# peterWon/LVI-ExC

Hardware: AMD Instinct MI355X
Metric: M residual+Jacobian evals/s per GN iter (higher is better)
Workload: dtype f64; 1 GPU; config4-full-LVI: 1000000 surfel + 200000 IMU samples (gyro+accel blocks) + 49992 ORB reprojection blocks, 25023 knots @ dt=0.02; step = residuals + analytic Jacobians + Huber + J^T J/J^T r assembly (no linear solve); n_tangent=155259, bandwidth=179, n_border=52, tracks=orb, parallelism=sequence-per-gpu x1, allreduce_transport=none (one sequence)

## Files before the change

### lvi-exc_amd/csrc/lvx_eval.hip

```cpp
#include <algorithm>
#include <cmath>
#include <cstring>
#include <functional>
#include <numeric>
#include <cstdlib>

#include <thread>
#include "lvx_ctx.h"
#include "lvx_fold.h"

namespace lvx {

#define LVX_PW 4
struct Keys { int k0, k1, lm; };
LVX_HD bool same(const Keys& a, const Keys& b) { return a.k0 == b.k0 && a.k1 == b.k1 && a.lm == b.lm; }

struct Cal { ImuCal imu; SensorCal lidar, cam; const double* rho; };
__device__ __forceinline__ Cal load_cal(const DevCommon& cm) {
  const double* s = cm.state + 7 * (size_t)cm.N;
  Cal c;
  c.imu.tau = s[7]; c.imu.roll = s[8]; c.imu.pitch = s[9]; c.imu.ba = load_v3(s + 10); c.imu.bg = load_v3(s + 13);
  c.lidar.q = load_q(s + 16); c.lidar.p = load_v3(s + 20); c.lidar.tau = s[23];
  c.cam.q = load_q(s + 24); c.cam.p = load_v3(s + 28); c.cam.tau = s[31];
  c.rho = s + 32;
// ... 277 lines not shown
      for (int a = 0; a < NR; ++a) {
        int32_t* jc = cm.jcols + (orow + a) * LVX_JAC_WIDTH;
        double* jv = cm.jvals + (orow + a) * LVX_JAC_WIDTH;
#pragma unroll
        for (int c = 0; c < NC; ++c) {
          const int g = fam.col(c, key, cm.N);
          const bool dead = tangent_locked(g, cm.N, cm.L, cm.locks);
          jc[c] = dead ? -1 : g;
          jv[c] = dead ? 0.0 : J[a][c];
        }
        for (int c = NC; c < LVX_JAC_WIDTH; ++c) { jc[c] = -1; jv[c] = 0.0; }
      }
    }
    if (scale != 1.0) {
#pragma unroll
      for (int a = 0; a < NR; ++a) {
        r[a] *= scale;
#pragma unroll
        for (int c = 0; c < NC; ++c) J[a][c] *= scale;
      }
    }
  }
  mycost = wave_sum(mycost);
  if (lane == 0) atomicAdd(&cm.cost[rep], mycost);
  if (cm.what & LVX_EVAL_NORMAL_EQ) {
#pragma unroll
    for (int a = 0; a < NR; ++a) {
      rs[lane * NR + a] = valid ? r[a] : 0.0;
#pragma unroll
      for (int c = 0; c < NC; ++c) Jt[c * TS + lane * NR + a] = valid ? J[a][c] : 0.0;
    }
    Keys pk;
    pk.k0 = __shfl_up(key.k0, 1); pk.k1 = __shfl_up(key.k1, 1); pk.lm = __shfl_up(key.lm, 1);
    const bool head = (lane == 0) || !same(pk, key);
    const unsigned long long heads = __ballot(head);
    const int myseg = __popcll(heads & ((2ull << lane) - 1ull)) - 1;
    if (head) { seg_l0[myseg] = lane; seg_ok[myseg] = valid ? 1 : 0; seg_keys[myseg] = key; }
    if (lane == 0) nseg_s = __popcll(heads);
  }
  }
  if (!(cm.what & LVX_EVAL_NORMAL_EQ)) return;
  __syncthreads();
  const int nseg = nseg_s;
  const int tid = threadIdx.x;
  constexpr int NT = 64 * PW;
  for (int e = tid; e < nseg * NC; e += NT) { const int sg = e / NC, c = e % NC; cpos[e] = seg_ok[sg] ? cm.ord[fam.col(c, seg_keys[sg], cm.N)] : LVX_DEAD; }
  constexpr int ITER = (NP + NC + NT - 1) / NT;
  unsigned code[ITER];
#pragma unroll
  for (int i = 0; i < ITER; ++i) { const int p = tid + NT * i; code[i] = p < NP ? pairs[p] : 0u; }
  __syncthreads();
  for (int sg = 0; sg < nseg; ++sg) {
    if (!seg_ok[sg]) continue;
    const int l0 = seg_l0[sg];
    const int l1 = sg + 1 < nseg ? seg_l0[sg + 1] : 64;
    const int rb = l0 * NR, re = l1 * NR;
    const int* cp = &cpos[sg * NC];
#pragma unroll
    for (int i = 0; i < ITER; ++i) {
      const int p = tid + NT * i;
      if (p < NP) {
        const int a = code[i] & 0xff, b = code[i] >> 8;
        const int pa = cp[a], pb = cp[b];
        if (pa == LVX_DEAD || pb == LVX_DEAD) continue;
        const double* ja = &Jt[a * TS];
        const double* jb = &Jt[b * TS];
        double acc = 0.0;
        for (int row = rb; row < re; ++row) acc += ja[row] * jb[row];
        if (a != b && pa == pb) acc *= 2.0;
        add_H(cm, pa, pb, acc, rep);
      } else if (p < NP + NC) {
        const int c = p - NP;
        const int pc = cp[c];
        if (pc == LVX_DEAD) continue;
        const double* jc = &Jt[c * TS];
        double acc = 0.0;
        for (int row = rb; row < re; ++row) acc += jc[row] * rs[row];
        add_g(cm, pc, acc, rep);
      }
    }
  }
}

__device__ void hub_eval_thread(const DevCommon& cm, double t_map, int want_surf, int want_cs, HubShared* hubs, int s) {
  if (s > 1) return;
  if ((s == 0 && !want_surf) || (s == 1 && !want_cs)) { hubs[s].ok = 0; return; }
#ifdef LVX_KTIME_FOLD
  long long kt_[5] = {0, 0, 0, 0, 0}; long long kt0_ = __builtin_amdgcn_s_memtime(); const long long kts_ = kt0_;
#define HKT(i) { const long long n_ = __builtin_amdgcn_s_memtime(); kt_[i] += n_ - kt0_; kt0_ = n_; }
#else
#define HKT(i)
#endif
  const SplineRef sp{cm.t0, cm.dt, cm.N, cm.state, cm.state + 3 * (size_t)cm.N};
  const Cal cal = load_cal(cm);
  const bool tl = s == 0 ? (cm.locks & LVX_LOCK_LIDAR_TAU) != 0 : (cm.locks & LVX_LOCK_CAM_TAU) != 0;
  const double tau = s == 0 ? cal.lidar.tau : cal.cam.tau;
  double s1[1][2]; hub_spans(t_map, tl, cm.sensor_mto, s1);
  HKT(0)
  Segs sg; KnotRef kh; hubs[s].ok = 0;
  if (!build_segments(sp, s1, 1, &sg)) return;
  if (!seg_lookup(sp, sg, t_map + tau, &kh)) return;
  HKT(1)
  if (!(tl ? pose_eval<true>(sp, kh, &hubs[s].A) : pose_eval<true, true>(sp, kh, &hubs[s].A))) { hubs[s].ok = -RES_NONUNIT; return; }
  HKT(2)
  hub_matrix(hubs[s].A, hubs[s].M);
  hubs[s].ok = 1;
  HKT(3)
#ifdef LVX_KTIME_FOLD
  printf("HKT hub set %d: cal+spans %lld segments+lookup %lld pose_eval %lld hub_matrix+stores %lld | total %lld, ends at %lld (ticks of s_memtime)\n", s, kt_[0], kt_[1], kt_[2], kt_[3],
         (long long)__builtin_amdgcn_s_memtime() - kts_, (long long)__builtin_amdgcn_s_memtime());
#endif
}
__device__ __forceinline__ void state_prepass_block(const DevCommon& cm, So3Pre* tab, int nblk_tab, double t_map, int want_surf, int want_cs, HubShared* hubs, int blk) {
  if (blk >= nblk_tab) { hub_eval_thread(cm, t_map, want_surf, want_cs, hubs, threadIdx.x); return; }
  const int k = blk * blockDim.x + threadIdx.x;
  if (k >= cm.N) return;
  const double* so3 = cm.state + 3 * (size_t)cm.N;
  So3Pre e;
  if (k + 1 < cm.N) so3_pre(load_q(so3 + 4 * (size_t)k), load_q(so3 + 4 * (size_t)(k + 1)), &e);
  else { e.Om = mk(0, 0, 0); e.on = 0.0; e.Jri = m3_identity(); e.c3 = 1.0 / 12.0; e.ok = 1; }
  tab[k] = e;
}

struct Aux { int wid, xk, lm; const PreWin* pw; };
struct GyroAcc {
  enum { PMAJ = 1 };
  enum { NK = 12, NG = 3, NR = 3, HUB = -1, KPK = 3, LVO = 3, WS = 1, GL = 32, SKIP_GG = 0, SECONDARY = 0, LB = 64, NCP = 15, USE_PRE = 1, OCC = 1, FAM = LVX_FAM_GYRO };
  __device__ static constexpr int jm(int c) { return c; }
  int n; const double* t; const double* m3; const int* perm; double weight, huber;
  __device__ int eval(const DevCommon& cm, const SplineRef& sp, const Cal& cal, const HubShared*, int si, double r[NR], double (*J)[NCP], int& key, Aux& aux) const {
    return gyro_residual<true, true>(sp, cal.imu, t[si], load_v3(m3 + 3 * (size_t)si), weight, &key, r, J, aux.pw);
  }
  __device__ static int klv(int c) { return 6 * (c / 3) + 3 + c % 3; }
  __device__ static int gcol(int g, int N, int nt) { return 6 * N + 5 + g; }
  __device__ void put(const DevCommon& cm, const HubShared*, int si, bool valid, int key, const double (*J)[NCP]) const {
    if (!valid) { put_skipped(cm, FAM, perm[si]); return; }
    put_record<NR, GYRO_NC>(cm, FAM, perm[si], key, -1, -1, [&](int a, int c) { return J[a][c]; });
  }
};
#ifndef LVX_SURF_WS
#define LVX_SURF_WS 3
#endif
template <bool TAU> struct SurfAccT {
  enum { DEPG = LVX_SURF_WS >= 3 ? 3 : 0 };
  enum { NK = 24, NG = 12 + (TAU ? 1 : 0), NR = 1, HUB = 0, KPK = 6, LVO = 0, WS = LVX_SURF_WS, GL = 16, SKIP_GG = 0, SECONDARY = 0, LB = 64, NCP = 36 + (TAU ? 1 : 0), USE_PRE = 1, OCC = 2, FAM = LVX_FAM_SURFEL };
  __device__ static constexpr int jm(int c) { return c; }
  int n; const double* t; const double* pt; const double* rowpl; const int* perm; double t_map, weight, huber;
  struct Row { double t; v3 p, Pi; };
  enum { PREFETCH = 1 };
  __device__ Row load(int si) const { return Row{t[si], load_v3(pt + 3 * (size_t)si), load_v3(rowpl + 3 * (size_t)si)}; }
  __device__ int eval_row(const DevCommon& cm, const SplineRef& sp, const Cal& cal, const HubShared* hub, const Row& row, double r[NR], double (*J)[NCP], int& key, Aux& aux) const {
    const bool tl = (cm.locks & LVX_LOCK_LIDAR_TAU) != 0;
    const double tk = row.t;
    Segs segs;
    if (tl) {
      KnotRef kr;
      const int st = two_point_lookup(sp, t_map, tk, tk + cal.lidar.tau, &kr);
      if (st >= 0) {
        if (st == 1) return RES_RANGE;
        if (hub->ok != 1) return hub->ok < 0 ? RES_NONUNIT : RES_RANGE;
        if (st == 2) return RES_RANGE;
        LVX_KT(aux.pw, 8)
        return surfel_residual_pseudo<true, TAU>(sp, hub->A, segs, cal.lidar, tk, row.p, row.Pi, weight, &key, r, J, aux.pw, &kr);
      }
    }
    const double pad = tl ? 0.0 : cm.sensor_mto;
    const double spans[2][2] = {{t_map - pad, t_map + pad}, {tk - pad, tk + pad}};
    if (!build_segments(sp, spans, 2, &segs)) return RES_RANGE;
    KnotRef kh;
    if (!seg_lookup(sp, segs, t_map + cal.lidar.tau, &kh)) return RES_RANGE;
    if (hub->ok != 1) return hub->ok < 0 ? RES_NONUNIT : RES_RANGE;
    if (kh.i0 != hub->A.k.i0 || kh.u != hub->A.k.u) return LVX_ERR_FALLBACK;
    LVX_KT(aux.pw, 8)
    return surfel_residual_pseudo<true, TAU>(sp, hub->A, segs, cal.lidar, tk, row.p, row.Pi, weight, &key, r, J, aux.pw);
  }
  __device__ static int klv(int c) { return c; }
  __device__ static int gcol(int g, int N, int nt) { return g < 6 ? nt + g : 6 * N + 8 + (g - 6); }
  __device__ void put(const DevCommon& cm, const HubShared* hub, int si, bool valid, int key, const double (*J)[NCP]) const {
    if (!valid) { put_skipped(cm, FAM, perm[si]); return; }
    put_record<NR, SURF_NC + (TAU ? 1 : 0)>(cm, FAM, perm[si], hub->A.k.i0, key, -1, [&](int a, int c) { return c < 24 ? hub_col(*hub, &J[a][24], c) : (c < 48 ? J[a][c - 24] : J[a][c - 18]); });
  }
};
using SurfAcc = SurfAccT<false>;
template <bool TAU> struct CamSurfAccT {
  enum { NK = 24, NG = 18 + (TAU ? 1 : 0), NR = 1, HUB = 1, KPK = 6, LVO = 0, WS = 1, GL = 16, SKIP_GG = 0, SECONDARY = 0, LB = 64, NCP = 42 + (TAU ? 1 : 0), USE_PRE = 1, OCC = 2, FAM = LVX_FAM_CAMSURF };
  __device__ static constexpr int jm(int c) { return c; }
  int n; const int* lm; const int* plane; const int* perm; const double* planes; const double* lm_uv; const double* lm_t0; double t_map, weight, huber;
  __device__ int eval(const DevCommon& cm, const SplineRef& sp, const Cal& cal, const HubShared* hub, int si, double r[NR], double (*J)[NCP], int& key, Aux& aux) const {
    const bool tl = (cm.locks & LVX_LOCK_CAM_TAU) != 0;
    const int l = lm[si];
    const double tk = lm_t0[l];
    Segs segs;
    if (tl) {
      KnotRef kr;
      const int st = two_point_lookup(sp, t_map, tk, tk + cal.cam.tau, &kr);
      if (st >= 0) {
        if (st == 1) return RES_RANGE;
// ... 140 lines not shown
#pragma unroll
        for (int c = 0; c < 12; ++c) v[c] = src[(size_t)c * n];
      }
      const int k0 = in ? k0r : -1, k1 = in ? k1r : -1;
      const bool live = in && k1 >= 0;
      const int o0 = k0 - 4 * w0, o1 = k1 - 4 * w1;
      const bool stray = live && (o0 < 0 || o0 > 3 || o1 < 0 || o1 > 3);
      const bool valid = live && !stray;
#pragma unroll
      for (int c = 0; c < 12; ++c) v[c] = live ? v[c] : 0.0;
      for (int e = lane; e < 2 * BR * LDP; e += 64) Pr[e] = 0.0;
      __builtin_amdgcn_fence(__ATOMIC_RELEASE, "wavefront");
      __builtin_amdgcn_wave_barrier();
      {
        double* dst = (side ? Po : Pr) + (2 * b + a) * LDP + 6 * (side ? o1 : o0) + 12 * h;
        if (valid) {
#pragma unroll
          for (int c = 0; c < 12; ++c) dst[c] = v[c];
        }
      }
      __builtin_amdgcn_fence(__ATOMIC_RELEASE, "wavefront");
      __builtin_amdgcn_wave_barrier();
      __builtin_amdgcn_fence(__ATOMIC_ACQUIRE, "wavefront");
      const int nks = (2 * min(8, m1 - base) + 3) >> 2;
      for (int ks = 0; ks < nks; ++ks) {
        double fr[3], fo[3];
#pragma unroll
        for (int c = 0; c < 3; ++c) { fr[c] = Pr[ks * 4 * LDP + frag_off + c * 16]; fo[c] = Po[ks * 4 * LDP + frag_off + c * 16]; }
#pragma unroll
        for (int ci = 0; ci < 3; ++ci)
#pragma unroll
          for (int cj = 0; cj < 3; ++cj) D[ci * 3 + cj] = __builtin_amdgcn_mfma_f64_16x16x4f64(fr[ci], fo[cj], D[ci * 3 + cj], 0, 0, 0);
      }
      {
        unsigned long long sm = __ballot(stray && part == 0);
        while (sm) {
          const int sl = __ffsll((long long)sm) - 1; sm &= sm - 1;
          const int sb = sl >> 3;
          const int sk0 = __shfl(k0, sl), sk1 = __shfl(k1, sl);
          __builtin_amdgcn_wave_barrier();
          if (b == sb) {
#pragma unroll
            for (int c = 0; c < 12; ++c) sbuf[wv][a][24 * side + 12 * h + c] = v[c];
          }
          __builtin_amdgcn_fence(__ATOMIC_RELEASE, "wavefront");
          __builtin_amdgcn_wave_barrier();
          __builtin_amdgcn_fence(__ATOMIC_ACQUIRE, "wavefront");
          for (int e2 = lane; e2 < 576; e2 += 64) {
            const int x = e2 / 24, y = e2 % 24;
            const double val = sbuf[wv][0][x] * sbuf[wv][0][24 + y] + sbuf[wv][1][x] * sbuf[wv][1][24 + y];
            if (val == 0.0) continue;
            const int pa = cm.ord[6 * (sk0 + x / 6) + x % 6], pb = cm.ord[6 * (sk1 + y / 6) + y % 6];
            if (pa == LVX_DEAD || pb == LVX_DEAD) continue;
            add_H(cm, pa, pb, pa == pb ? 2.0 * val : val, rep);
          }
          __builtin_amdgcn_fence(__ATOMIC_RELEASE, "wavefront");
          __builtin_amdgcn_wave_barrier();
        }
      }
      __builtin_amdgcn_fence(__ATOMIC_RELEASE, "wavefront");
      __builtin_amdgcn_wave_barrier();
    }
    int pcol[3], prow[12];
#pragma unroll
    for (int cj = 0; cj < 3; ++cj) { const int y = cj * 16 + (lane & 15); pcol[cj] = y < 42 ? cm.ord[24 * w1 + y] : LVX_DEAD; }
#pragma unroll
    for (int ci = 0; ci < 3; ++ci)
#pragma unroll
      for (int vv = 0; vv < 4; ++vv) { const int x = ci * 16 + (lane >> 4) + 4 * vv; prow[ci * 4 + vv] = x < 42 ? cm.ord[24 * w0 + x] : LVX_DEAD; }
#pragma unroll
    for (int ci = 0; ci < 3; ++ci)
#pragma unroll
      for (int cj = 0; cj < 3; ++cj)
#pragma unroll
        for (int vv = 0; vv < 4; ++vv) {
          const double val = D[ci * 3 + cj][vv];
          const int pa = prow[ci * 4 + vv], pb = pcol[cj];
          if (val == 0.0 || pa == LVX_DEAD || pb == LVX_DEAD) continue;
          add_H(cm, pa, pb, pa == pb ? 2.0 * val : val, rep);
        }
  }
}

struct RepLmRows { const double* T; const int* k; int n; const int* ptr; const int* rows; int L; };
template <bool TAU>
__global__ __launch_bounds__(256) void k_reproj_lmrows(RepLmRows q, DevCommon cm) {
  constexpr int RW = 56 + (TAU ? 1 : 0);
  extern __shared__ double rowbuf[];
  const int wv = threadIdx.x >> 6, lane = threadIdx.x & 63;
  const int l = blockIdx.x * 4 + wv;
  if (l >= q.L) return;
  double* rb = rowbuf + (size_t)wv * cm.lm_ls;
  for (int k = lane; k < cm.lm_ls; k += 64) rb[k] = 0.0;
  const int j0 = q.ptr[l], j1 = q.ptr[l + 1], p0 = cm.lm_p0[l], N = cm.N;
  __builtin_amdgcn_fence(__ATOMIC_RELEASE, "wavefront");
  __builtin_amdgcn_wave_barrier();
  for (int jb = j0; jb < j1; jb += 4) {
    double val[4]; int pc[4];
#pragma unroll
    for (int u = 0; u < 4; ++u) {
      val[u] = 0.0; pc[u] = LVX_DEAD;
      if (jb + u < j1 && lane < RW) {
        const int i = q.rows[jb + u];
        const int kr = q.k[i], ko = q.k[(size_t)q.n + i];
        if (ko >= 0) {
          val[u] = q.T[(size_t)i * RW + lane];
          const int c = lane < 24 ? lane : lane - 24;
          pc[u] = lane < 48 ? cm.ord[6 * ((lane < 24 ? kr : ko) + c / 6) + c % 6] : (lane < 54 ? cm.ord[6 * N + 15 + (lane - 48)] : (lane < 56 ? LVX_LM_BASE : cm.ord[6 * N + 21]));
        }
      }
    }
#pragma unroll
    for (int u = 0; u < 4; ++u) {
      if (pc[u] == LVX_DEAD || val[u] == 0.0) continue;
      int slot;
      if (lane == 54 || lane == 55) slot = cm.lm_wl + cm.nbd + (lane - 54);
      else if (pc[u] >= 0) { slot = pc[u] - p0; if (slot < 0 || slot >= cm.lm_wl) { atomicOr(cm.err, 4); continue; } }
      else slot = cm.lm_wl + (-1 - pc[u]);
      atomicAdd(&rb[slot], val[u]);
    }
  }
  __builtin_amdgcn_fence(__ATOMIC_RELEASE, "wavefront");
  __builtin_amdgcn_wave_barrier();
  __builtin_amdgcn_fence(__ATOMIC_ACQUIRE, "wavefront");
  double* row = cm.lmH + (size_t)l * cm.lm_ls;
  for (int k = lane; k < cm.lm_ls; k += 64) row[k] = rb[k];
}

struct RepFused { const int* g_start; const int* g_count; int ng; };
#define RF_LDP 97
#define RF_WBUF (32 * RF_LDP + 48)
template <bool TAU>
__global__ __launch_bounds__(256, 1) void k_reproj_fused(ReprojFamT<TAU> fam, RepFused q, DevCommon cm, long long row0) {
  constexpr int RJ = REP_NC + (TAU ? 1 : 0), LDP = RF_LDP, TCOL = 90, RCOL = 91, LCOL = 92;
  __shared__ double smf[4 * RF_WBUF];
  const int lane = threadIdx.x & 63, wv = threadIdx.x >> 6;
  const int N = cm.N;
  const bool want_ne = (cm.what & LVX_EVAL_NORMAL_EQ) != 0;
  const bool lm_free = want_ne && cm.L > 0 && !(cm.locks & LVX_LOCK_LANDMARKS);
  double* P = smf + wv * RF_WBUF;
  int* posL = (int*)(P + 32 * LDP);
  for (int g = blockIdx.x * 4 + wv; g < q.ng; g += gridDim.x * 4) {
    const int rep = g % cm.nrep;
    const int si = q.g_start[g] + lane;
    const bool in = lane < q.g_count[g];
    double r[2], J[2][RJ];
    Keys key{-1, -1, -1};
    bool valid = false;
    double mycost = 0.0;
    if (in) {
      const SplineRef sp{cm.t0, cm.dt, cm.N, cm.state, cm.state + 3 * (size_t)cm.N};
      const Cal cal = load_cal(cm);
      const int status = fam.eval_pre(cm, sp, cal, si, r, J, key);
      if (status == RES_OUTSIDE) fallback_row(cm, LVX_FAM_REPROJ, si);
      else if (status != RES_OK) atomicOr(cm.err, status);
      else {
        valid = true;
        double scale;
        mycost = 0.5 * huber_rho(fam.huber, r[0] * r[0] + r[1] * r[1], &scale);
        if (cm.residuals) { const long long orow = row0 + (long long)fam.perm[si] * 2; cm.residuals[orow] = r[0]; cm.residuals[orow + 1] = r[1]; }
        if (scale != 1.0) {
#pragma unroll
          for (int a = 0; a < 2; ++a) {
            r[a] *= scale;
#pragma unroll
            for (int c = 0; c < RJ; ++c) J[a][c] *= scale;
          }
        }
      }
    }
    mycost = wave_sum(mycost);
    if (lane == 0 && mycost != 0.0) atomicAdd(&cm.cost[rep], mycost);
#ifdef RF_EVAL_ONLY
    if (cm.N > 0) continue;
#endif
    if (!want_ne) continue;
    const int my_w0 = valid ? key.k0 >> 2 : -1, my_w1 = valid ? key.k1 >> 2 : -1;
    const int my_o0 = 6 * (key.k0 & 3), my_o1 = 48 + 6 * (key.k1 & 3);
    const int my_p0 = (valid && lm_free) ? cm.lm_p0[key.lm] : 0;
    unsigned long long rem = __ballot(valid);
    while (rem) {
      const int lf = __ffsll((long long)rem) - 1;
      const int w0 = __builtin_amdgcn_readfirstlane(__shfl(my_w0, lf)), w1 = __builtin_amdgcn_readfirstlane(__shfl(my_w1, lf));
      const unsigned long long wm = __ballot(valid && my_w0 == w0 && my_w1 == w1);
      rem &= ~wm;
      for (int c = lane; c < 96; c += 64) {
        int tg = -1;
        if (c < 42) { if (4 * w0 + c / 6 < N) tg = 24 * w0 + c; }
        else if (c < 48) tg = 6 * N + 15 + (c - 42);
        else if (c < 90) { if (4 * w1 + (c - 48) / 6 < N) tg = 24 * w1 + (c - 48); }
        else if (c == TCOL && TAU) tg = 6 * N + 21;
        posL[c] = tg >= 0 ? cm.ord[tg] : LVX_DEAD;
      }
      d4 D[21];
#pragma unroll
      for (int t = 0; t < 21; ++t) D[t] = d4{0.0, 0.0, 0.0, 0.0};
      unsigned long long todo = wm;
      while (todo) {
        const int l0 = __ffsll((long long)todo) - 1;
        const int ws = min(l0, 48);
        const unsigned long long chunk = todo & (0xffffull << ws);
        todo &= ~chunk;
// ... 2261 lines not shown
```

### lvi-exc_amd/csrc/lvx_resid.h

```cpp
#pragma once
#include "lvx_math.h"

namespace lvx {

struct SplineRef {
  double t0, dt;
  int n;
  const double* r3;
  const double* so3;
};

struct CamIntr {
  double fx, fy, cx, cy, k1, k2, p1, p2, k3, readout;
  double inv_K11, inv_K13, inv_K22, inv_K23;
  int rows, cols, do_distortion;
};

struct ImuCal { double roll, pitch; v3 ba, bg; double tau; };
struct SensorCal { quat q; v3 p; double tau; };

LVX_HD v3 load_v3(const double* p) { return mk(p[0], p[1], p[2]); }
LVX_HD quat load_q(const double* p) { quat q; q.x = p[0]; q.y = p[1]; q.z = p[2]; q.w = p[3]; return q; }

struct Segs { int nseg; int i1[2]; int n[2]; };
// ... 296 lines not shown
      J[a][51] = jp.x; J[a][52] = jp.y; J[a][53] = jp.z;
      if (TAU) J[a][LPOS_NC] = plane_tau_jac(hub, k, g);
    }
  }
  return RES_OK;
}

enum { SURFP_NC = 36 };
struct PoseVal { v3 p; double Bp[4]; quat c[4]; So3Val s; };
LVX_HD int pose_value_pre(const SplineRef& sp, const KnotRef& k, const So3Pre* pre, PoseVal* out) {
  R3Basis b; r3_basis(k.u, sp.dt, &b);
  v3 p = mk(0, 0, 0);
#pragma unroll
  for (int j = 0; j < 4; ++j) { out->Bp[j] = b.Bp[j]; p = p + b.Bp[j] * load_v3(sp.r3 + 3 * (k.i0 + j)); }
  out->p = p;
  load_so3_cp(sp, k.i0, out->c);
  return so3_value_pre(out->c, pre, k.u, &out->s);
}
LVX_HD void pose_pull_to_knots(const PoseVal& e, const So3Pre* pre, v3 gpos, v3 gxi, double* J24) {
  v3 y[4];
  so3_pullback_pre(e.c, pre, e.s, gxi, y);
#pragma unroll
  for (int j = 0; j < 4; ++j) {
    J24[6 * j + 0] = e.Bp[j] * gpos.x; J24[6 * j + 1] = e.Bp[j] * gpos.y; J24[6 * j + 2] = e.Bp[j] * gpos.z;
    J24[6 * j + 3] = y[j].x; J24[6 * j + 4] = y[j].y; J24[6 * j + 5] = y[j].z;
  }
}

template <bool PRE>
LVX_HD int pose_twist(const SplineRef& sp, const KnotRef& k, const So3Pre* pre, v3* v, v3* w_body) {
  R3Basis b; r3_basis(k.u, sp.dt, &b);
  v3 vv = mk(0, 0, 0);
#pragma unroll
  for (int j = 0; j < 4; ++j) vv = vv + b.Bv[j] * load_v3(sp.r3 + 3 * (k.i0 + j));
  *v = vv;
  quat c[4]; load_so3_cp(sp, k.i0, c);
  So3Eval e;
  if (PRE) { const int bad = so3_eval_pre<true, false, false>(c, pre, k.u, sp.dt, &e); if (bad) return bad; }
  else if (!so3_eval<true, false, false>(c, k.u, sp.dt, &e)) return 1;
  *w_body = e.w_body;
  return 0;
}
template <bool PRE = false, bool TAU = false>
LVX_HD int surfel_residual_pseudo(const SplineRef& sp, const PoseEval& hub, const Segs& segs, const SensorCal& lidar, double t_k, v3 p_L, v3 Pi,
                                  double weight, int* i0_k, double r[1], double J[1][SURFP_NC + (TAU ? 1 : 0)], const PreWin* pw = nullptr, const KnotRef* kr_in = nullptr) {
  KnotRef kr;
  if (kr_in) kr = *kr_in;
  else if (!seg_lookup(sp, segs, t_k + lidar.tau, &kr)) return RES_RANGE;
  *i0_k = kr.i0;
  PoseEval k;
  PoseVal kv;
  const So3Pre* pre = PRE ? pre_at(*pw, kr.i0) : nullptr;
  if (PRE && !pre) return RES_OUTSIDE;
  LVX_KT(pw, 9)
  if (PRE) { const int bad = pose_value_pre(sp, kr, pre, &kv); if (bad) return (bad & 1) ? RES_NONUNIT : RES_OUTSIDE; k.p = kv.p; k.so3.q = kv.s.q; }
  else if (!pose_eval<true, false, false>(sp, kr, &k)) return RES_NONUNIT;
  LVX_KT(pw, 10)
  const v3 pLr = qrot(lidar.q, p_L);
  const v3 p_I = pLr + lidar.p;
  PlaneChain pc; plane_chain(hub, k, lidar, p_I, Pi, &pc);
  r[0] = weight * pc.r_unweighted;
  const PlaneGrads g = plane_grads(hub, pc, p_I, weight);
  LVX_KT(pw, 11)
  if (PRE) pose_pull_to_knots(kv, pre, g.gp, g.gxk, &J[0][0]); else pose_to_knots(k, g.gp, g.gxk, &J[0][0]);
  LVX_KT(pw, 12)
  J[0][24] = -g.gp.x; J[0][25] = -g.gp.y; J[0][26] = -g.gp.z; J[0][27] = g.gx0.x; J[0][28] = g.gx0.y; J[0][29] = g.gx0.z;
  const v3 jq = (2.0 * weight) * (cross(pc.nL, pc.x) - cross(pc.m, pLr));
  const v3 jp = weight * (pc.m - pc.nL);
  J[0][30] = jq.x; J[0][31] = jq.y; J[0][32] = jq.z; J[0][33] = jp.x; J[0][34] = jp.y; J[0][35] = jp.z;
  if (TAU) {
    v3 vk, wk;
    const int bad = pose_twist<PRE>(sp, kr, pre, &vk, &wk);
    if (bad) return (bad & 1) ? RES_NONUNIT : RES_OUTSIDE;
    J[0][SURFP_NC] = dot(g.gp, vk - hub.v) + dot(g.gx0, hub.so3.w_body) + dot(g.gxk, wk);
  }
  return RES_OK;
}
LVX_HD void hub_matrix(const PoseEval& h, double M[6][24]) {
  for (int a = 0; a < 6; ++a) for (int c = 0; c < 24; ++c) M[a][c] = 0.0;
  for (int j = 0; j < 4; ++j) {
    for (int a = 0; a < 3; ++a) M[a][6 * j + a] = h.Bp[j];
    for (int a = 0; a < 3; ++a) for (int b = 0; b < 3; ++b) M[3 + a][6 * j + 3 + b] = h.so3.dxi[j].a[3 * a + b];
  }
}

LVX_HD void cam_distortion(const CamIntr& c, double x, double y, double* dx, double* dy, double D[4]) {
  const double mx2 = x * x, my2 = y * y, mxy = x * y, rho2 = mx2 + my2;
  const double rad = c.k1 * rho2 + c.k2 * rho2 * rho2 + c.k3 * rho2 * rho2 * rho2;
  *dx = x * rad + 2.0 * c.p1 * mxy + c.p2 * (rho2 + 2.0 * mx2);
  *dy = y * rad + 2.0 * c.p2 * mxy + c.p1 * (rho2 + 2.0 * my2);
  if (D) {
    const double drad = c.k1 + 2.0 * c.k2 * rho2 + 3.0 * c.k3 * rho2 * rho2;
    D[0] = rad + x * drad * 2.0 * x + 2.0 * c.p1 * y + c.p2 * (2.0 * x + 4.0 * x);
    D[1] = x * drad * 2.0 * y + 2.0 * c.p1 * x + c.p2 * (2.0 * y);
    D[2] = y * drad * 2.0 * x + 2.0 * c.p2 * y + c.p1 * (2.0 * x);
    D[3] = rad + y * drad * 2.0 * y + 2.0 * c.p2 * x + c.p1 * (2.0 * y + 4.0 * y);
  }
}
LVX_HD v3 cam_unproject(const CamIntr& c, double u, double v) {
  if (c.do_distortion) {
    const double mx_d = c.inv_K11 * u + c.inv_K13, my_d = c.inv_K22 * v + c.inv_K23;
    double dx, dy;
    cam_distortion(c, mx_d, my_d, &dx, &dy, nullptr);
    double mx_u = mx_d - dx, my_u = my_d - dy;
    for (int i = 1; i < 8; ++i) { cam_distortion(c, mx_u, my_u, &dx, &dy, nullptr); mx_u = mx_d - dx; my_u = my_d - dy; }
    return mk(mx_u, my_u, 1.0);
  }
  const double invdet = 1.0 / (c.fx * c.fy);
  return mk((c.fy * invdet) * u + ((-c.cx * c.fy) * invdet), (c.fx * invdet) * v + ((-(c.fx * c.cy)) * invdet), (c.fx * c.fy) * invdet);
}
LVX_HD void cam_project(const CamIntr& c, v3 X, double y[2], double G[2][3]) {
  const double z = 1e-32 + X.z;
  const double pu0 = X.x / z, pu1 = X.y / z;
  double pd0 = pu0, pd1 = pu1;
  double D[4] = {1.0, 0.0, 0.0, 1.0};
  if (c.do_distortion) {
    double dx, dy, Dd[4];
    cam_distortion(c, pu0, pu1, &dx, &dy, Dd);
    pd0 = pu0 + dx; pd1 = pu1 + dy;
    D[0] = 1.0 + Dd[0]; D[1] = Dd[1]; D[2] = Dd[2]; D[3] = 1.0 + Dd[3];
  }
  y[0] = c.fx * pd0 + c.cx;
  y[1] = c.fy * pd1 + c.cy;
  if (G) {
    const double iz = 1.0 / z;
    const double a0[3] = {iz, 0.0, -pu0 * iz}, a1[3] = {0.0, iz, -pu1 * iz};
    for (int k = 0; k < 3; ++k) {
      G[0][k] = c.fx * (D[0] * a0[k] + D[1] * a1[k]);
      G[1][k] = c.fy * (D[2] * a0[k] + D[3] * a1[k]);
    }
  }
}

enum { REP_NC = 55, REP_NR = 2 };
template <bool NEED_J, bool TAU = false>
LVX_HD int reproj_residual(const SplineRef& sp, const CamIntr& ci, const SensorCal& cam, bool tau_locked, double max_time_offset,
                           double u_ref, double v_ref, double t0_ref, double u_obs, double v_obs, double t0_obs, double rho, double weight,
                           int* i0_ref, int* i0_obs, double r[2], double J[2][REP_NC + (TAU ? 1 : 0)], const So3Pre* gpre = nullptr) {
  double t1, t2;
  if (t0_ref <= t0_obs) { t1 = t0_ref; t2 = t0_obs; } else { t1 = t0_obs; t2 = t0_ref; }
  if (!tau_locked) { t1 -= max_time_offset; t2 += max_time_offset; }
  const double margin = 1e-3;
  const double spans[2][2] = {{t1 - margin, t1 + ci.readout + margin}, {t2 - margin, t2 + ci.readout + margin}};
  Segs segs;
  if (!build_segments(sp, spans, 2, &segs)) return RES_RANGE;
  const double row_delta = ci.readout / (double)ci.rows;
  const double t_ref = madd_2r(v_ref, row_delta, t0_ref + cam.tau);
  const double t_obs = madd_2r(v_obs, row_delta, t0_obs + cam.tau);
  KnotRef kr, ko;
  if (!seg_lookup(sp, segs, t_ref, &kr)) return RES_RANGE;
  if (!seg_lookup(sp, segs, t_obs, &ko)) return RES_RANGE;
  *i0_ref = kr.i0; *i0_obs = ko.i0;
  PoseEval er, eo;
  if (!TAU && gpre) {
    const int bad = pose_eval_pre<NEED_J>(sp, kr, &er, gpre + kr.i0) | pose_eval_pre<NEED_J>(sp, ko, &eo, gpre + ko.i0);
    if (bad) return (bad & 1) ? RES_NONUNIT : RES_OUTSIDE;
  } else {
    if (!pose_eval<NEED_J, TAU>(sp, kr, &er)) return RES_NONUNIT;
    if (!pose_eval<NEED_J, TAU>(sp, ko, &eo)) return RES_NONUNIT;
  }
  const v3 p_ct = qrot_inv(cam.q, -cam.p);
  const v3 yh = cam_unproject(ci, u_ref, v_ref);
  const v3 X_ref = qrot(cam.q, yh - rho * p_ct);
  const v3 X = qrot(er.so3.q, X_ref) + rho * er.p;
  const v3 X_obs = qrot_inv(eo.so3.q, X - rho * eo.p);
  const v3 X_c = qrot_inv(cam.q, X_obs) + rho * p_ct;
// ... 184 lines not shown
```

Baseline: 2854 Mevals/s.

## Spread hub pose evaluation across a wavefront and batch landmark-row index loads

The hub pose evaluation, which ran on one thread per sensor, is split across lanes of a wavefront. Each lane computes one knot pair's rotation terms, and the stages are separated by wave-level LDS syncs, with the 6x24 hub matrix written cooperatively. Separately, the landmark-row assembly kernel loads 64 row indices and knot keys per lane at once, broadcasts them with readlane, and processes 16 rows per unrolled group while hoisting lane-constant ordering lookups. The aim is to shorten the serial critical path of the prepass and cut redundant scalar loads in the landmark kernel, at the cost of more registers and extra LDS syncs.

New measurement: 2909 Mevals/s (median of 6 runs). +1.9%, better.

```diff
diff --git a/lvi-exc_amd/csrc/lvx_eval.hip b/lvi-exc_amd/csrc/lvx_eval.hip
--- a/lvi-exc_amd/csrc/lvx_eval.hip
+++ b/lvi-exc_amd/csrc/lvx_eval.hip
@@ -383,9 +383,25 @@
   }
 }
 
-__device__ void hub_eval_thread(const DevCommon& cm, double t_map, int want_surf, int want_cs, HubShared* hubs, int s) {
+__device__ __forceinline__ void wave_sync_lds() {
+  __builtin_amdgcn_fence(__ATOMIC_RELEASE, "wavefront");
+  __builtin_amdgcn_wave_barrier();
+  __builtin_amdgcn_fence(__ATOMIC_ACQUIRE, "wavefront");
+}
+template <bool NEED_V> __device__ __forceinline__ bool hub_pose_wave(const SplineRef& sp, const KnotRef& kh, int lane, HubLanes* X, HubShared* h) {
+  hub_lanes_pairs<NEED_V>(sp, kh, lane, X, &h->A);
+  wave_sync_lds();
+  if (!hub_lanes_ok(X)) return false;
+  hub_lanes_coefs(lane, X);
+  wave_sync_lds();
+  hub_lanes_knots<NEED_V>(lane, X, &h->A);
+  wave_sync_lds();
+  return true;
+}
+__device__ void hub_eval_wave(const DevCommon& cm, double t_map, int want_surf, int want_cs, HubShared* hubs, int s, int lane) {
+  __shared__ HubLanes xs[2];
   if (s > 1) return;
-  if ((s == 0 && !want_surf) || (s == 1 && !want_cs)) { hubs[s].ok = 0; return; }
+  if ((s == 0 && !want_surf) || (s == 1 && !want_cs)) { if (lane == 0) hubs[s].ok = 0; return; }
 #ifdef LVX_KTIME_FOLD
   long long kt_[5] = {0, 0, 0, 0, 0}; long long kt0_ = __builtin_amdgcn_s_memtime(); const long long kts_ = kt0_;
 #define HKT(i) { const long long n_ = __builtin_amdgcn_s_memtime(); kt_[i] += n_ - kt0_; kt0_ = n_; }
@@ -398,22 +414,24 @@
   const double tau = s == 0 ? cal.lidar.tau : cal.cam.tau;
   double s1[1][2]; hub_spans(t_map, tl, cm.sensor_mto, s1);
   HKT(0)
-  Segs sg; KnotRef kh; hubs[s].ok = 0;
-  if (!build_segments(sp, s1, 1, &sg)) return;
-  if (!seg_lookup(sp, sg, t_map + tau, &kh)) return;
+  Segs sg; KnotRef kh;
+  if (!build_segments(sp, s1, 1, &sg) || !seg_lookup(sp, sg, t_map + tau, &kh)) { if (lane == 0) hubs[s].ok = 0; return; }
   HKT(1)
-  if (!(tl ? pose_eval<true>(sp, kh, &hubs[s].A) : pose_eval<true, true>(sp, kh, &hubs[s].A))) { hubs[s].ok = -RES_NONUNIT; return; }
+  if (!(tl ? hub_pose_wave<false>(sp, kh, lane, &xs[s], &hubs[s]) : hub_pose_wave<true>(sp, kh, lane, &xs[s], &hubs[s]))) {
+    if (lane == 0) hubs[s].ok = -RES_NONUNIT;
+    return;
+  }
   HKT(2)
-  hub_matrix(hubs[s].A, hubs[s].M);
-  hubs[s].ok = 1;
+  hub_lanes_matrix(lane, &xs[s], hubs[s].M);
+  if (lane == 0) hubs[s].ok = 1;
   HKT(3)
 #ifdef LVX_KTIME_FOLD
-  printf("HKT hub set %d: cal+spans %lld segments+lookup %lld pose_eval %lld hub_matrix+stores %lld | total %lld, ends at %lld (ticks of s_memtime)\n", s, kt_[0], kt_[1], kt_[2], kt_[3],
-         (long long)__builtin_amdgcn_s_memtime() - kts_, (long long)__builtin_amdgcn_s_memtime());
+  if (lane == 0) printf("HKT hub set %d: cal+spans %lld segments+lookup %lld pose_eval %lld hub_matrix+stores %lld | total %lld, ends at %lld (ticks of s_memtime)\n", s, kt_[0], kt_[1], kt_[2], kt_[3],
+                        (long long)__builtin_amdgcn_s_memtime() - kts_, (long long)__builtin_amdgcn_s_memtime());
 #endif
 }
 __device__ __forceinline__ void state_prepass_block(const DevCommon& cm, So3Pre* tab, int nblk_tab, double t_map, int want_surf, int want_cs, HubShared* hubs, int blk) {
-  if (blk >= nblk_tab) { hub_eval_thread(cm, t_map, want_surf, want_cs, hubs, threadIdx.x); return; }
+  if (blk >= nblk_tab) { hub_eval_wave(cm, t_map, want_surf, want_cs, hubs, threadIdx.x >> 6, threadIdx.x & 63); return; }
   const int k = blk * blockDim.x + threadIdx.x;
   if (k >= cm.N) return;
   const double* so3 = cm.state + 3 * (size_t)cm.N;
@@ -720,42 +738,46 @@
   }
 }
 
+constexpr int LMR_G = 16;
 struct RepLmRows { const double* T; const int* k; int n; const int* ptr; const int* rows; int L; };
 template <bool TAU>
 __global__ __launch_bounds__(256) void k_reproj_lmrows(RepLmRows q, DevCommon cm) {
   constexpr int RW = 56 + (TAU ? 1 : 0);
   extern __shared__ double rowbuf[];
-  const int wv = threadIdx.x >> 6, lane = threadIdx.x & 63;
+  const int wv = __builtin_amdgcn_readfirstlane(threadIdx.x >> 6), lane = threadIdx.x & 63;
   const int l = blockIdx.x * 4 + wv;
   if (l >= q.L) return;
+  const int j0 = q.ptr[l], j1 = q.ptr[l + 1], p0 = cm.lm_p0[l], N = cm.N;
+  const int pc_fix = lane < 48 ? LVX_DEAD : (lane < 54 ? cm.ord[6 * N + 15 + (lane - 48)] : (lane < 56 ? LVX_LM_BASE : (lane < RW ? cm.ord[6 * N + 21] : LVX_DEAD)));
+  const int c24 = lane < 24 ? lane : lane - 24;
   double* rb = rowbuf + (size_t)wv * cm.lm_ls;
   for (int k = lane; k < cm.lm_ls; k += 64) rb[k] = 0.0;
-  const int j0 = q.ptr[l], j1 = q.ptr[l + 1], p0 = cm.lm_p0[l], N = cm.N;
   __builtin_amdgcn_fence(__ATOMIC_RELEASE, "wavefront");
   __builtin_amdgcn_wave_barrier();
-  for (int jb = j0; jb < j1; jb += 4) {
-    double val[4]; int pc[4];
-#pragma unroll
-    for (int u = 0; u < 4; ++u) {
-      val[u] = 0.0; pc[u] = LVX_DEAD;
-      if (jb + u < j1 && lane < RW) {
-        const int i = q.rows[jb + u];
-        const int kr = q.k[i], ko = q.k[(size_t)q.n + i];
-        if (ko >= 0) {
-          val[u] = q.T[(size_t)i * RW + lane];
-          const int c = lane < 24 ? lane : lane - 24;
-          pc[u] = lane < 48 ? cm.ord[6 * ((lane < 24 ? kr : ko) + c / 6) + c % 6] : (lane < 54 ? cm.ord[6 * N + 15 + (lane - 48)] : (lane < 56 ? LVX_LM_BASE : cm.ord[6 * N + 21]));
-        }
-      }
-    }
-#pragma unroll
-    for (int u = 0; u < 4; ++u) {
-      if (pc[u] == LVX_DEAD || val[u] == 0.0) continue;
-      int slot;
-      if (lane == 54 || lane == 55) slot = cm.lm_wl + cm.nbd + (lane - 54);
-      else if (pc[u] >= 0) { slot = pc[u] - p0; if (slot < 0 || slot >= cm.lm_wl) { atomicOr(cm.err, 4); continue; } }
-      else slot = cm.lm_wl + (-1 - pc[u]);
-      atomicAdd(&rb[slot], val[u]);
+  for (int jc = j0; jc < j1; jc += 64) {
+    const int nc = min(64, j1 - jc);
+    int bi = 0, bkr = 0, bko = -1;
+    if (lane < nc) { bi = q.rows[jc + lane]; bkr = q.k[bi]; bko = q.k[(size_t)q.n + bi]; }
+    for (int g0 = 0; g0 < nc; g0 += LMR_G) {
+      double val[LMR_G]; int pc[LMR_G];
+#pragma unroll
+      for (int u = 0; u < LMR_G; ++u) {
+        val[u] = 0.0; pc[u] = LVX_DEAD;
+        if (g0 + u >= nc) continue;
+        const int i = __builtin_amdgcn_readlane(bi, g0 + u), kr = __builtin_amdgcn_readlane(bkr, g0 + u), ko = __builtin_amdgcn_readlane(bko, g0 + u);
+        if (ko < 0 || lane >= RW) continue;
+        val[u] = q.T[(size_t)i * RW + lane];
+        pc[u] = lane < 48 ? cm.ord[6 * (lane < 24 ? kr : ko) + c24] : pc_fix;
+      }
+#pragma unroll
+      for (int u = 0; u < LMR_G; ++u) {
+        if (pc[u] == LVX_DEAD || val[u] == 0.0) continue;
+        int slot;
+        if (lane == 54 || lane == 55) slot = cm.lm_wl + cm.nbd + (lane - 54);
+        else if (pc[u] >= 0) { slot = pc[u] - p0; if (slot < 0 || slot >= cm.lm_wl) { atomicOr(cm.err, 4); continue; } }
+        else slot = cm.lm_wl + (-1 - pc[u]);
+        atomicAdd(&rb[slot], val[u]);
+      }
     }
   }
   __builtin_amdgcn_fence(__ATOMIC_RELEASE, "wavefront");
diff --git a/lvi-exc_amd/csrc/lvx_resid.h b/lvi-exc_amd/csrc/lvx_resid.h
--- a/lvi-exc_amd/csrc/lvx_resid.h
+++ b/lvi-exc_amd/csrc/lvx_resid.h
@@ -402,6 +402,88 @@
     for (int a = 0; a < 3; ++a) M[a][6 * j + a] = h.Bp[j];
     for (int a = 0; a < 3; ++a) for (int b = 0; b < 3; ++b) M[3 + a][6 * j + 3 + b] = h.so3.dxi[j].a[3 * a + b];
   }
+}
+
+struct HubLanes { quat c[4], E[4]; double B[4], dB[4], Bp[4]; v3 d[4]; m3 R[4], Jri[4], P[4], T[4], dxi[4]; int ok[4]; };
+
+template <bool NEED_V>
+LVX_HD void hub_lanes_pairs(const SplineRef& sp, const KnotRef& k, int lane, HubLanes* X, PoseEval* out) {
+  if (lane < 3) {
+    const int j = lane + 1;
+    const double u = k.u, u2 = u * u, u3 = u2 * u;
+    const double B1 = 5.0 / 6.0 + u * (3.0 / 6.0) + u2 * (-3.0 / 6.0) + u3 * (1.0 / 6.0), B2 = 1.0 / 6.0 + u * (3.0 / 6.0) + u2 * (3.0 / 6.0) + u3 * (-2.0 / 6.0), B3 = u3 * (1.0 / 6.0);
+    const double Bj = j == 1 ? B1 : (j == 2 ? B2 : B3);
+    X->B[j] = Bj;
+    if (NEED_V) {
+      const double di = 1.0 / sp.dt;
+      const double U1 = di, U2 = di * (2.0 * u), U3 = di * (3.0 * u2);
+      const double dB1 = U1 * (3.0 / 6.0) + U2 * (-3.0 / 6.0) + U3 * (1.0 / 6.0), dB2 = U1 * (3.0 / 6.0) + U2 * (3.0 / 6.0) + U3 * (-2.0 / 6.0), dB3 = U3 * (1.0 / 6.0);
+      X->dB[j] = j == 1 ? dB1 : (j == 2 ? dB2 : dB3);
+    }
+    bool ok = true;
+    const v3 Om = logq_half(qmul(qconj(load_q(sp.so3 + 4 * (k.i0 + j - 1))), load_q(sp.so3 + 4 * (k.i0 + j))), &ok);
+    const v3 d = 2.0 * Om;
+    const quat E = expq_half(Bj * Om);
+    X->d[j] = d; X->E[j] = E; X->R[j] = rotmat(E); X->ok[j] = ok ? 1 : 0;
+    X->Jri[j] = so3_Jr_inv(d);
+    X->P[j] = Bj * so3_Jr(Bj * d);
+  } else if (lane == 3) {
+    out->k = k;
+    R3Basis b; r3_basis(k.u, sp.dt, &b);
+    v3 p = mk(0, 0, 0), v = mk(0, 0, 0);
+    for (int j = 0; j < 4; ++j) {
+      const v3 cj = load_v3(sp.r3 + 3 * (k.i0 + j));
+      out->Bp[j] = b.Bp[j]; X->Bp[j] = b.Bp[j]; p = p + b.Bp[j] * cj;
+      if (NEED_V) v = v + b.Bv[j] * cj;
+      X->c[j] = load_q(sp.so3 + 4 * (k.i0 + j));
+    }
+    out->p = p;
+    if (NEED_V) out->v = v;
+  }
+}
+LVX_HD bool hub_lanes_ok(const HubLanes* X) { return X->ok[1] && X->ok[2] && X->ok[3]; }
+
+LVX_HD void hub_lanes_coefs(int lane, HubLanes* X) {
+  if (lane < 3) {
+    const int j = lane + 1;
+    const m3 R3 = X->R[3];
+    const m3 R32t = tmul(R3, transpose(X->R[2]));
+    X->T[j] = (j == 1 ? R32t : (j == 2 ? transpose(R3) : m3_identity())) * X->P[j];
+  } else if (lane == 3) {
+    X->T[0] = tmul(X->R[1] * (X->R[2] * X->R[3]), m3_identity());
+  }
+}
+template <bool NEED_V>
+LVX_HD void hub_lanes_knots(int lane, HubLanes* X, PoseEval* out) {
+  if (lane >= 4) return;
+  const int k = lane;
+  const int ja = k == 0 ? 1 : k, jb = k == 3 ? 3 : k + 1;
+  m3 first = X->T[ja] * X->Jri[ja];
+  m3 second = mul_t(X->T[jb], X->Jri[jb]);
+  if (k == 0) first = X->T[0];
+  if (k == 3) second = m3_zero();
+  const m3 Xe = first - second;
+  const m3 r = 2.0 * mul_t(Xe, rotmat(X->c[k]));
+  out->so3.dxi[k] = r; X->dxi[k] = r;
+  if (lane == 0) {
+    quat q = X->c[0];
+    for (int j = 1; j < 4; ++j) q = qmul(q, X->E[j]);
+    out->so3.q = q;
+    if (NEED_V) {
+      const v3 w1 = X->dB[1] * X->d[1];
+      const v3 w2 = tmulv(X->R[2], w1) + X->dB[2] * X->d[2];
+      out->so3.w_body = tmulv(X->R[3], w2) + X->dB[3] * X->d[3];
+    }
+  }
+}
+
+LVX_HD double hub_lanes_entry(const HubLanes* X, int e) {
+  const int a = e / 24, c = e - 24 * a, j = c / 6, m = c - 6 * j;
+  if (a < 3) return m == a ? X->Bp[j] : 0.0;
+  return m >= 3 ? X->dxi[j].a[3 * (a - 3) + (m - 3)] : 0.0;
+}
+LVX_HD void hub_lanes_matrix(int lane, const HubLanes* X, double M[6][24]) {
+  for (int e = lane; e < 144; e += 64) M[e / 24][e % 24] = hub_lanes_entry(X, e);
 }
 
 LVX_HD void cam_distortion(const CamIntr& c, double x, double y, double* dx, double* dy, double D[4]) {
```
